# jason2714/de-i2i-gan

Hardware: AMD Instinct MI355X
Metric: paired 256x256 images/sec (G+D train step) (higher is better)
Workload: dtype bf16

## Files before the change

de-i2i-gan_amd/csrc/elementwise.hip:

```cpp
#include <hip/hip_runtime.h>
#include <algorithm>
#include <math.h>

#include "../../include/dei2i_hip.h"
#include "launch.h"

namespace dei2i {

template <typename T>
__global__ void nchw_to_nhwc_kernel(const float* __restrict__ src, T* __restrict__ dst, int N, int C, int hs, int ws, int H,
                                    int W, int Cs) {
  constexpr int VEC = Elem<T>::VEC;
  const int cv = Cs / VEC;
  const size_t total = (size_t)N * H * W * cv;
  for (size_t i = (size_t)blockIdx.x * blockDim.x + threadIdx.x; i < total; i += (size_t)gridDim.x * blockDim.x) {
    const size_t hw = (size_t)H * W;
    const size_t p = i % hw;
    size_t r = i / hw;
    const int v = (int)(r % cv);
    const int n = (int)(r / cv);
    const int h = (int)(p / W), w = (int)(p % W);
    const int sy = (int)(((long long)h * hs) / H), sx = (int)(((long long)w * ws) / W);
    float f[VEC];
#pragma unroll
// ... 54 lines not shown
    }
    const u32x4 pk = Elem<T>::pack(f);
    *reinterpret_cast<u32x4*>(out + i * VEC) = pk;
    if constexpr (sizeof(T) == 2) {
      if (out8 != nullptr) store_e4m3_of_bf16x8(out8 + i * 8, pk, scale8);
    }
  }
}

template <typename T>
__global__ void affine_act_img_kernel(const T* __restrict__ x, const float* __restrict__ A, const float* __restrict__ B,
                                      T* __restrict__ out, size_t nvec_img, int cv, float slope) {
  constexpr int VEC = Elem<T>::VEC;
  const int n = blockIdx.y;
  const size_t base = (size_t)n * nvec_img;
  float av[VEC], bv[VEC];
  size_t i = (size_t)blockIdx.x * blockDim.x + threadIdx.x;
  const int c = (int)(i % cv) * VEC;
  ldcoef<VEC>(A + (size_t)n * cv * VEC + c, av);
  ldcoef<VEC>(B + (size_t)n * cv * VEC + c, bv);
  for (; i < nvec_img; i += (size_t)gridDim.x * blockDim.x) {
    float f[VEC];
    Elem<T>::unpack(*reinterpret_cast<const u32x4*>(x + (base + i) * VEC), f);
#pragma unroll
    for (int e = 0; e < VEC; ++e) {
      const float v = fmaf(av[e], f[e], bv[e]);
      f[e] = fmaf(slope, fminf(v, 0.f), fmaxf(v, 0.f));
    }
    *reinterpret_cast<u32x4*>(out + (base + i) * VEC) = Elem<T>::pack(f);
  }
}


template <typename T>
__global__ void spade_act_kernel(const T* __restrict__ x, const float* __restrict__ mean, const float* __restrict__ rstd,
                                 const T* __restrict__ gb, T* __restrict__ out, int N, int H, int W, int C, int up,
                                 int gb_mode, unsigned char* __restrict__ out8, float scale8) {
  constexpr int VEC = Elem<T>::VEC;
  const int cv = C / VEC;
  const int Hs = H >> up, Ws = W >> up;
  const size_t total = (size_t)N * H * W * cv;
  for (size_t i = (size_t)blockIdx.x * blockDim.x + threadIdx.x; i < total; i += (size_t)gridDim.x * blockDim.x) {
    const int c = (int)(i % cv) * VEC;
    size_t r = i / cv;
    const int w = (int)(r % W); r /= W;
    const int h = (int)(r % H);
    const int n = (int)(r / H);
    float xv[VEC], gm[VEC], bt[VEC];
    Elem<T>::unpack(*reinterpret_cast<const u32x4*>(x + (((size_t)n * Hs + (h >> up)) * Ws + (w >> up)) * C + c), xv);
    size_t gpix;
    if (gb_mode == 0) gpix = ((size_t)n * H + h) * W + w;
    else gpix = ((size_t)n * 5 + border_class(h, H)) * 5 + border_class(w, W);
    Elem<T>::unpack(*reinterpret_cast<const u32x4*>(gb + gpix * 2 * C + c), gm);
    Elem<T>::unpack(*reinterpret_cast<const u32x4*>(gb + gpix * 2 * C + C + c), bt);
    float o[VEC], mv[VEC], rv[VEC];
    ldcoef<VEC>(mean + (size_t)n * C + c, mv);
    ldcoef<VEC>(rstd + (size_t)n * C + c, rv);
#pragma unroll
    for (int e = 0; e < VEC; ++e) {
      const float xh = (xv[e] - mv[e]) * rv[e];
      const float v = fmaf(xh, 1.f + gm[e], bt[e]);
      o[e] = v > 0.f ? v : 0.f;
    }
    const u32x4 pk = Elem<T>::pack(o);
    *reinterpret_cast<u32x4*>(out + i * VEC) = pk;
    if constexpr (sizeof(T) == 2) {
      if (out8 != nullptr) store_e4m3_of_bf16x8(out8 + i * 8, pk, scale8);
    }
  }
}

template <typename T>
__global__ void act_bwd_kernel(const T* __restrict__ dz, const T* __restrict__ z, T* __restrict__ g, size_t nvec, int act) {
  constexpr int VEC = Elem<T>::VEC;
  for (size_t i = (size_t)blockIdx.x * blockDim.x + threadIdx.x; i < nvec; i += (size_t)gridDim.x * blockDim.x) {
    float d[VEC], zz[VEC];
    Elem<T>::unpack(*reinterpret_cast<const u32x4*>(dz + i * VEC), d);
    Elem<T>::unpack(*reinterpret_cast<const u32x4*>(z + i * VEC), zz);
#pragma unroll
    for (int e = 0; e < VEC; ++e) d[e] *= act_grad_from_out(zz[e], act);
    *reinterpret_cast<u32x4*>(g + i * VEC) = Elem<T>::pack(d);
  }
}

template <typename T>
__global__ void compose_fwd_kernel(const T* __restrict__ raw, const float* __restrict__ x_in, float* __restrict__ out,
                                   float* __restrict__ prob, int N, int HW, int Cs) {
  const size_t total = (size_t)N * HW;
  for (size_t i = (size_t)blockIdx.x * blockDim.x + threadIdx.x; i < total; i += (size_t)gridDim.x * blockDim.x) {
    const size_t n = i / HW, p = i % HW;
    const T* rp = raw + i * Cs;
    const float pr = 1.f / (1.f + expf(-Elem<T>::load(rp + 3)));
    prob[i] = pr;
#pragma unroll
    for (int c = 0; c < 3; ++c) {
      const float fg = tanhf(Elem<T>::load(rp + c));
      const size_t o = (n * 3 + c) * HW + p;
      out[o] = x_in[o] * (1.f - pr) + fg * pr;
    }
  }
}

// ... 195 lines not shown
    else hipLaunchKernelGGL((affine_act_kernel<float, false>), dim3(grid, groups), dim3(256), 0, st, (const float*)x, a, b, (const float*)res, (float*)out, nvec, cv, act, o8, e4m3_scale);
  }
  return (int)hipGetLastError();
}

int dei2i_affine_act_img_fwd(int dtype, int N, int HW, int C, const void* x, const float* A, const float* B, float slope, void* out,
                             dei2i_stream s) {
  const int vec = vec_of(dtype);
  if (N <= 0 || HW <= 0 || C <= 0 || C % vec || !x || !A || !B || !out) return DEI2I_ERR_BAD_ARG;
  const int cv = C / vec;
  if (256 % cv != 0 && cv % 256 != 0) return DEI2I_ERR_BAD_ARG;
  const size_t nvec_img = (size_t)HW * cv;
  unsigned blocks = (unsigned)std::min<size_t>((nvec_img + 255) / 256, 512);
  if (cv > 256) blocks = (blocks / (cv / 256)) * (cv / 256);
  if (blocks < 1) blocks = cv > 256 ? cv / 256 : 1;
  if (dtype == DT_BF16)
    hipLaunchKernelGGL(affine_act_img_kernel<bf16_t>, dim3(blocks, N), dim3(256), 0, (hipStream_t)s, (const bf16_t*)x, A, B, (bf16_t*)out,
                       nvec_img, cv, slope);
  else
    hipLaunchKernelGGL(affine_act_img_kernel<float>, dim3(blocks, N), dim3(256), 0, (hipStream_t)s, (const float*)x, A, B, (float*)out,
                       nvec_img, cv, slope);
  return (int)hipGetLastError();
}

int dei2i_spade_act_fwd(int dtype, int N, int H, int W, int C, int up, const void* x, const float* mean, const float* rstd,
                        const void* gb, int gb_mode, void* out, void* out_e4m3, float e4m3_scale, dei2i_stream s) {
  const int vec = vec_of(dtype);
  if (N <= 0 || H <= 0 || W <= 0 || C <= 0 || C % vec || up < 0 || up > 1 || !x || !mean || !rstd || !gb || !out)
    return DEI2I_ERR_BAD_ARG;
  if (out_e4m3 != nullptr && (dtype != DT_BF16 || !(e4m3_scale > 0.f))) return DEI2I_ERR_BAD_ARG;
  unsigned char* o8 = (unsigned char*)out_e4m3;
  if (up && ((H | W) & 1)) return DEI2I_ERR_BAD_ARG;
  if (gb_mode == 1 && (H < 4 || W < 4)) return DEI2I_ERR_BAD_ARG;
  const size_t total = (size_t)N * H * W * (C / vec);
  if (dtype == DT_BF16)
    hipLaunchKernelGGL(spade_act_kernel<bf16_t>, dim3(grid_for(total, 256, EW_CAP)), dim3(256), 0, (hipStream_t)s,
                       (const bf16_t*)x, mean, rstd, (const bf16_t*)gb, (bf16_t*)out, N, H, W, C, up, gb_mode, o8, e4m3_scale);
  else
    hipLaunchKernelGGL(spade_act_kernel<float>, dim3(grid_for(total, 256, EW_CAP)), dim3(256), 0, (hipStream_t)s,
                       (const float*)x, mean, rstd, (const float*)gb, (float*)out, N, H, W, C, up, gb_mode, o8, e4m3_scale);
  return (int)hipGetLastError();
}

int dei2i_act_bwd(int dtype, size_t n, const void* dz, const void* z, int act, void* g, dei2i_stream s) {
  const int vec = vec_of(dtype);
  if (n == 0 || n % vec || !dz || !z || !g) return DEI2I_ERR_BAD_ARG;
  const size_t nvec = n / vec;
  if (dtype == DT_BF16)
    hipLaunchKernelGGL(act_bwd_kernel<bf16_t>, dim3(grid_for(nvec, 256, EW_CAP)), dim3(256), 0, (hipStream_t)s,
                       (const bf16_t*)dz, (const bf16_t*)z, (bf16_t*)g, nvec, act);
  else
    hipLaunchKernelGGL(act_bwd_kernel<float>, dim3(grid_for(nvec, 256, EW_CAP)), dim3(256), 0, (hipStream_t)s,
                       (const float*)dz, (const float*)z, (float*)g, nvec, act);
  return (int)hipGetLastError();
}

int dei2i_compose_fwd(int dtype, int N, int H, int W, int Cs, const void* raw, const float* x_in, float* out, float* prob,
                      dei2i_stream s) {
  if (N <= 0 || H <= 0 || W <= 0 || Cs < 4 || Cs % vec_of(dtype) || !raw || !x_in || !out || !prob) return DEI2I_ERR_BAD_ARG;
  const size_t total = (size_t)N * H * W;
  if (dtype == DT_BF16)
    hipLaunchKernelGGL(compose_fwd_kernel<bf16_t>, dim3(grid_for(total, 256, EW_CAP)), dim3(256), 0, (hipStream_t)s,
                       (const bf16_t*)raw, x_in, out, prob, N, H * W, Cs);
  else
    hipLaunchKernelGGL(compose_fwd_kernel<float>, dim3(grid_for(total, 256, EW_CAP)), dim3(256), 0, (hipStream_t)s,
                       (const float*)raw, x_in, out, prob, N, H * W, Cs);
  return (int)hipGetLastError();
}

int dei2i_compose_bwd(int dtype, int N, int H, int W, int Cs, const void* raw, const float* x_in, const float* d_out,
                      const float* d_prob, void* d_raw, float* d_x, dei2i_stream s) {
  if (N <= 0 || H <= 0 || W <= 0 || Cs < 4 || Cs % vec_of(dtype) || !raw || !x_in || !d_raw) return DEI2I_ERR_BAD_ARG;
  const size_t total = (size_t)N * H * W;
// ... 66 lines not shown
```

de-i2i-gan_amd/csrc/reduce.hip:

```cpp
#include <hip/hip_runtime.h>
#include <math.h>

#include "../../include/dei2i_hip.h"
#include "launch.h"

namespace dei2i {

static inline int vec_of(int dtype) { return dtype == DT_BF16 ? 8 : 4; }

template <int NV, int VEC, typename OT = float>
DEI2I_D void block_combine_store(const float (&vals)[NV][VEC], int cv, int rpp, float* smem, OT* __restrict__ dst, int C) {
  const int tid = threadIdx.x;
  const int vcol = tid % cv, prow = tid / cv;
  __syncthreads();
  if (prow < rpp) {
#pragma unroll
    for (int q = 0; q < NV; ++q)
#pragma unroll
      for (int e = 0; e < VEC; ++e) smem[((q * VEC + e) * rpp + prow) * cv + vcol] = vals[q][e];
  }
  __syncthreads();
#pragma unroll 1
  for (int o = tid; o < NV * VEC * cv; o += 256) {
    const int qe = o / cv, vc = o - qe * cv;
    const float* src = smem + (size_t)qe * rpp * cv + vc;
    float sum = 0.f;
    for (int r = 0; r < rpp; ++r) sum += src[r * cv];
    const int q = qe / VEC, e = qe - q * VEC;
    Elem<OT>::store(dst + (size_t)q * C + vc * VEC + e, sum);
  }
}

template <typename T>
// ... 374 lines not shown
        const float xh = (xv[e] - mv[e]) * rv[e];
        const float g = fmaf(xh, 1.f + gm[e], bt[e]) > 0.f ? d[e] : slope * d[e];
        v[0][e] = fmaf(g, xh, v[0][e]);
        v[1][e] += g;
      }
    }
  }
  block_combine_store<2, VEC, T>(v, cv, rpp, smem, dgb_cls + (((size_t)n * 5 + cy) * 5 + cx) * 2 * C, C);
}

__global__ __launch_bounds__(256) void spade_bwd_finalize_kernel(const float* __restrict__ partial, int N, int chunks, int C,
                                                                 double count, float* __restrict__ coef,
                                                                 void* __restrict__ dgb_cls, int dtype) {
  const int c = blockIdx.x, n = blockIdx.y;
  double sq[4];
  combine_records<4>(partial, (size_t)n * chunks, chunks, C, c, sq);
  if (threadIdx.x != 0) return;
  coef[((size_t)n * 2 + 0) * C + c] = (float)(sq[0] / count);
  coef[((size_t)n * 2 + 1) * C + c] = (float)(sq[1] / count);
  if (dgb_cls != nullptr) {
    const size_t gpix = ((size_t)n * 5 + 2) * 5 + 2;
    if (dtype == DT_BF16) {
      bf16_t* o = (bf16_t*)dgb_cls;
      o[gpix * 2 * C + c] = f32_to_bf16((float)sq[2]);
      o[gpix * 2 * C + C + c] = f32_to_bf16((float)sq[3]);
    } else {
      float* o = (float*)dgb_cls;
      o[gpix * 2 * C + c] = (float)sq[2];
      o[gpix * 2 * C + C + c] = (float)sq[3];
    }
  }
}

template <typename T>
__global__ void spade_bwd_apply_kernel(const T* __restrict__ dz, const T* __restrict__ x, const float* __restrict__ mean,
                                       const float* __restrict__ rstd, const T* __restrict__ gb, int gb_mode,
                                       const float* __restrict__ coef, const T* __restrict__ addend, T* __restrict__ dx, int N,
                                       int H, int W, int C, int up, float slope = 0.f) {
  constexpr int VEC = Elem<T>::VEC;
  const int cv = C / VEC;
  const int Hs = H >> up, Ws = W >> up;
  const size_t total = (size_t)N * Hs * Ws * cv;
  const float cnt = (float)(1 << (2 * up));
  for (size_t i = (size_t)blockIdx.x * blockDim.x + threadIdx.x; i < total; i += (size_t)gridDim.x * blockDim.x) {
    const int c = (int)(i % cv) * VEC;
    size_t r = i / cv;
    const int ws = (int)(r % Ws); r /= Ws;
    const int hs = (int)(r % Hs);
    const int n = (int)(r / Hs);
    float acc[VEC], xv[VEC], xh[VEC], mv[VEC], rv[VEC], k1[VEC], k2[VEC];
    ldcoef<VEC>(mean + (size_t)n * C + c, mv);
    ldcoef<VEC>(rstd + (size_t)n * C + c, rv);
    Elem<T>::unpack(*reinterpret_cast<const u32x4*>(x + i * VEC), xv);
#pragma unroll
    for (int e = 0; e < VEC; ++e) { acc[e] = 0.f; xh[e] = (xv[e] - mv[e]) * rv[e]; }
    for (int a = 0; a < (1 << up); ++a)
      for (int b = 0; b < (1 << up); ++b) {
        const int h = (hs << up) + a, w = (ws << up) + b;
        const size_t opix = ((size_t)n * H + h) * W + w;
        const size_t gpix = gb_mode == 0 ? opix : ((size_t)n * 5 + border_class(h, H)) * 5 + border_class(w, W);
        float d[VEC], gm[VEC], bt[VEC];
        Elem<T>::unpack(*reinterpret_cast<const u32x4*>(dz + opix * C + c), d);
        Elem<T>::unpack(*reinterpret_cast<const u32x4*>(gb + gpix * 2 * C + c), gm);
        Elem<T>::unpack(*reinterpret_cast<const u32x4*>(gb + gpix * 2 * C + C + c), bt);
#pragma unroll
        for (int e = 0; e < VEC; ++e) {
          const float g = fmaf(xh[e], 1.f + gm[e], bt[e]) > 0.f ? d[e] : slope * d[e];
          acc[e] = fmaf(g, 1.f + gm[e], acc[e]);
        }
      }
    float ad[VEC];
    if (addend != nullptr) Elem<T>::unpack(*reinterpret_cast<const u32x4*>(addend + i * VEC), ad);
    ldcoef<VEC>(coef + ((size_t)n * 2) * C + c, k1);
    ldcoef<VEC>(coef + ((size_t)n * 2 + 1) * C + c, k2);
#pragma unroll
    for (int e = 0; e < VEC; ++e) {
      float v = rv[e] * (acc[e] - cnt * k1[e] - cnt * xh[e] * k2[e]);
      if (addend != nullptr) v += ad[e];
      acc[e] = v;
    }
    *reinterpret_cast<u32x4*>(dx + i * VEC) = Elem<T>::pack(acc);
  }
}

template <typename T>
__global__ __launch_bounds__(256) void colsum_kernel(const T* __restrict__ g, float* __restrict__ partial, size_t rows, int C) {
  constexpr int VEC = Elem<T>::VEC;
  extern __shared__ float smem[];
  const int cv = C / VEC, rpp = 256 / cv;
  const int tid = threadIdx.x, vcol = tid % cv, prow = tid / cv;
  const size_t rows_per_block = (rows + gridDim.x - 1) / gridDim.x;
  const size_t rbeg = (size_t)blockIdx.x * rows_per_block;
  const size_t rend = rbeg + rows_per_block < rows ? rbeg + rows_per_block : rows;
  float v[1][VEC];
#pragma unroll
  for (int e = 0; e < VEC; ++e) v[0][e] = 0.f;
  if (prow < rpp) {
    const T* __restrict__ base = g + (size_t)vcol * VEC;
    auto acc = [&](const u32x4& q) {
      float f[VEC];
      Elem<T>::unpack(q, f);
#pragma unroll
      for (int e = 0; e < VEC; ++e) v[0][e] += f[e];
    };
    size_t r = rbeg + prow;
    for (; r + 3 * (size_t)rpp < rend; r += 4 * (size_t)rpp) {
      const u32x4 q0 = *reinterpret_cast<const u32x4*>(base + r * C);
      const u32x4 q1 = *reinterpret_cast<const u32x4*>(base + (r + rpp) * C);
      const u32x4 q2 = *reinterpret_cast<const u32x4*>(base + (r + 2 * (size_t)rpp) * C);
      const u32x4 q3 = *reinterpret_cast<const u32x4*>(base + (r + 3 * (size_t)rpp) * C);
      acc(q0); acc(q1); acc(q2); acc(q3);
    }
    for (; r < rend; r += rpp) acc(*reinterpret_cast<const u32x4*>(base + r * C));
  }
  block_combine_store<1, VEC>(v, cv, rpp, smem, partial + (size_t)blockIdx.x * C, C);
// ... 202 lines not shown
  if (ring == nullptr) return;
  const int H = Hs << up, W = Ws << up, cv = C / VEC;
  const int rp = ring_pixels(H, W);
  const int total = rp * cv;
  for (int i = blockIdx.x * 256 + tid; i < total; i += gridDim.x * 256) {
    const int r = i / cv, c = (i - r * cv) * VEC;
    int y, xx;
    ring_coord(r, H, W, y, xx);
    float xv[VEC], gm[VEC], bt[VEC], o[VEC];
    Elem<T>::unpack(*reinterpret_cast<const u32x4*>(x + (((size_t)n * Hs + (y >> up)) * Ws + (xx >> up)) * C + c), xv);
    const size_t gpix = ((size_t)n * 5 + prep_border_class(y, H)) * 5 + prep_border_class(xx, W);
    Elem<T>::unpack(*reinterpret_cast<const u32x4*>(gb + gpix * 2 * C + c), gm);
    Elem<T>::unpack(*reinterpret_cast<const u32x4*>(gb + gpix * 2 * C + C + c), bt);
#pragma unroll
    for (int e = 0; e < VEC; ++e) {
      const float xh = (xv[e] - smem[c + e]) * smem[C + c + e];
      const float v = fmaf(xh, 1.f + gm[e], bt[e]);
      o[e] = v > 0.f ? v : 0.f;
    }
    *reinterpret_cast<u32x4*>(ring + ((size_t)n * rp + r) * C + c) = Elem<T>::pack(o);
  }
}

}

using namespace dei2i;

static inline bool cv_ok(int dtype, int C) {
  const int vec = dtype == DT_BF16 ? 8 : 4;
  return C > 0 && C % vec == 0 && C / vec <= 256;
}
static inline size_t combine_lds(int dtype, int nv) { return (size_t)nv * (dtype == DT_BF16 ? 8 : 4) * 256 * sizeof(float); }

extern "C" {

int dei2i_moments_chunks(int HW) {
  int c = HW / 64;
  if (c < 1) c = 1;
  if (c > 64) c = 64;
  return c;
}

int dei2i_moments_partial(int dtype, int N, int HW, int C, const void* x, float* partial, dei2i_stream s) {
  if (N <= 0 || HW <= 0 || !cv_ok(dtype, C) || !x || !partial) return DEI2I_ERR_BAD_ARG;
  const int chunks = dei2i_moments_chunks(HW);
  if (dtype == DT_BF16)
    hipLaunchKernelGGL(moments_partial_kernel<bf16_t>, dim3(chunks, N), dim3(256), combine_lds(dtype, 2), (hipStream_t)s,
                       (const bf16_t*)x, partial, HW, C, chunks);
  else
    hipLaunchKernelGGL(moments_partial_kernel<float>, dim3(chunks, N), dim3(256), combine_lds(dtype, 2), (hipStream_t)s,
                       (const float*)x, partial, HW, C, chunks);
  return (int)hipGetLastError();
}

int dei2i_bn_finalize_train(int N, int HW, int C, const float* partial, const float* weight, const float* bias,
                            float* running_mean, float* running_var, float momentum, float eps, float* mean, float* rstd,
                            float* a, float* b, long long* num_batches_tracked, dei2i_stream s) {
  if (N <= 0 || HW <= 0 || C <= 0 || !partial || !weight || !bias || !mean || !rstd || !a || !b) return DEI2I_ERR_BAD_ARG;
  hipLaunchKernelGGL(bn_finalize_train_kernel, dim3(C), dim3(combine_threads(N * dei2i_moments_chunks(HW))), 0, (hipStream_t)s, partial, N,
                     dei2i_moments_chunks(HW), C, (double)N * (double)HW, weight, bias, running_mean, running_var, momentum,
                     eps, mean, rstd, a, b, num_batches_tracked, 0);
  return (int)hipGetLastError();
}

int dei2i_bn_finalize_train_chunks(int N, int HW, int C, int chunks, const float* partial, const float* weight, const float* bias,
                                   float* running_mean, float* running_var, float momentum, float eps, float* mean, float* rstd,
// ... 206 lines not shown
                       gb_mode == 0 ? (bf16_t*)dgb : (bf16_t*)nullptr, partial, H, W, C, up, chunks);
  else
    hipLaunchKernelGGL(spade_bwd_partial_kernel<float>, dim3(chunks, N), dim3(256), combine_lds(dtype, 4), st,
                       (const float*)dz, (const float*)x, mean, rstd, (const float*)gb, gb_mode,
                       gb_mode == 0 ? (float*)dgb : (float*)nullptr, partial, H, W, C, up, chunks);
  if (gb_mode == 1) {
    if (dtype == DT_BF16)
      hipLaunchKernelGGL(spade_bwd_border_kernel<bf16_t>, dim3(25, N), dim3(256), combine_lds(dtype, 2), st, (const bf16_t*)dz,
                         (const bf16_t*)x, mean, rstd, (const bf16_t*)gb, (bf16_t*)dgb, H, W, C, up);
    else
      hipLaunchKernelGGL(spade_bwd_border_kernel<float>, dim3(25, N), dim3(256), combine_lds(dtype, 2), st, (const float*)dz,
                         (const float*)x, mean, rstd, (const float*)gb, (float*)dgb, H, W, C, up);
  }
  return (int)hipGetLastError();
}

int dei2i_spade_bwd_border(int dtype, int N, int H, int W, int C, int up, const void* dz, const void* x, const float* mean,
                           const float* rstd, const void* gb, void* dgb_cls, dei2i_stream s) {
  if (N <= 0 || H < 4 || W < 4 || !cv_ok(dtype, C) || up < 0 || up > 1 || !dz || !x || !mean || !rstd || !gb || !dgb_cls)
    return DEI2I_ERR_BAD_ARG;
  hipStream_t st = (hipStream_t)s;
  if (dtype == DT_BF16)
    hipLaunchKernelGGL(spade_bwd_border_kernel<bf16_t>, dim3(25, N), dim3(256), combine_lds(dtype, 2), st, (const bf16_t*)dz,
                       (const bf16_t*)x, mean, rstd, (const bf16_t*)gb, (bf16_t*)dgb_cls, H, W, C, up);
  else
    hipLaunchKernelGGL(spade_bwd_border_kernel<float>, dim3(25, N), dim3(256), combine_lds(dtype, 2), st, (const float*)dz,
                       (const float*)x, mean, rstd, (const float*)gb, (float*)dgb_cls, H, W, C, up);
  return (int)hipGetLastError();
}

int dei2i_spade_bwd_apply(int dtype, int N, int H, int W, int C, int up, const void* dz, const void* x, const float* mean,
                          const float* rstd, const void* gb, int gb_mode, const float* partial, int chunks, void* dgb_cls,
                          float* coef, const void* addend, void* dx, dei2i_stream s) {
  const int vec = dtype == DT_BF16 ? 8 : 4;
  if (N <= 0 || H <= 0 || W <= 0 || !cv_ok(dtype, C) || up < 0 || up > 1 || !dz || !x || !mean || !rstd || !gb || !partial ||
      !coef || !dx)
    return DEI2I_ERR_BAD_ARG;
  hipStream_t st = (hipStream_t)s;
  hipLaunchKernelGGL(spade_bwd_finalize_kernel, dim3(C, N), dim3(combine_threads(chunks)), 0, st, partial, N, chunks, C,
                     (double)H * (double)W, coef, dgb_cls, dtype);
  const size_t total = (size_t)N * (H >> up) * (W >> up) * (C / vec);
  const unsigned grid = grid_for(total, 256, 256u * 16u);
  if (dtype == DT_BF16)
    hipLaunchKernelGGL(spade_bwd_apply_kernel<bf16_t>, dim3(grid), dim3(256), 0, st, (const bf16_t*)dz, (const bf16_t*)x, mean,
                       rstd, (const bf16_t*)gb, gb_mode, (const float*)coef, (const bf16_t*)addend, (bf16_t*)dx, N, H, W, C, up);
  else
    hipLaunchKernelGGL(spade_bwd_apply_kernel<float>, dim3(grid), dim3(256), 0, st, (const float*)dz, (const float*)x, mean,
                       rstd, (const float*)gb, gb_mode, (const float*)coef, (const float*)addend, (float*)dx, N, H, W, C, up);
  return (int)hipGetLastError();
}

int dei2i_in_act_bwd(int dtype, int N, int H, int W, int C, const void* dz, const void* x, const float* mean, const float* rstd,
                     float slope, const void* zero_table, float* partial, float* coef, const void* addend, void* dx, dei2i_stream s) {
  const int vec = dtype == DT_BF16 ? 8 : 4;
  if (N <= 0 || H < 4 || W < 4 || !cv_ok(dtype, C) || !dz || !x || !mean || !rstd || !zero_table || !partial || !coef || !dx)
    return DEI2I_ERR_BAD_ARG;
  hipStream_t st = (hipStream_t)s;
  const int chunks = dei2i_moments_chunks(H * W);
  if (dtype == DT_BF16)
    hipLaunchKernelGGL(spade_bwd_partial_kernel<bf16_t>, dim3(chunks, N), dim3(256), combine_lds(dtype, 4), st, (const bf16_t*)dz,
                       (const bf16_t*)x, mean, rstd, (const bf16_t*)zero_table, 1, (bf16_t*)nullptr, partial, H, W, C, 0, chunks, slope);
  else
    hipLaunchKernelGGL(spade_bwd_partial_kernel<float>, dim3(chunks, N), dim3(256), combine_lds(dtype, 4), st, (const float*)dz,
                       (const float*)x, mean, rstd, (const float*)zero_table, 1, (float*)nullptr, partial, H, W, C, 0, chunks, slope);
  hipLaunchKernelGGL(spade_bwd_finalize_kernel, dim3(C, N), dim3(combine_threads(chunks)), 0, st, (const float*)partial, N, chunks, C,
                     (double)H * (double)W, coef, (void*)nullptr, dtype);
  const size_t total = (size_t)N * H * W * (C / vec);
  const unsigned grid = grid_for(total, 256, 256u * 16u);
  if (dtype == DT_BF16)
    hipLaunchKernelGGL(spade_bwd_apply_kernel<bf16_t>, dim3(grid), dim3(256), 0, st, (const bf16_t*)dz, (const bf16_t*)x, mean, rstd,
                       (const bf16_t*)zero_table, 1, (const float*)coef, (const bf16_t*)addend, (bf16_t*)dx, N, H, W, C, 0, slope);
  else
    hipLaunchKernelGGL(spade_bwd_apply_kernel<float>, dim3(grid), dim3(256), 0, st, (const float*)dz, (const float*)x, mean, rstd,
                       (const float*)zero_table, 1, (const float*)coef, (const float*)addend, (float*)dx, N, H, W, C, 0, slope);
  return (int)hipGetLastError();
}

int dei2i_in_affine_act_bwd(int dtype, int N, int H, int W, int C, const void* dz, const void* x, const float* mean,
                            const float* rstd, float slope, const void* gb_table, void* dgb_table, float* partial, float* coef,
                            const void* addend, void* dx, dei2i_stream s) {
  const int vec = dtype == DT_BF16 ? 8 : 4;
  if (N <= 0 || H < 4 || W < 4 || !cv_ok(dtype, C) || !dz || !x || !mean || !rstd || !gb_table || !dgb_table || !partial || !coef || !dx)
    return DEI2I_ERR_BAD_ARG;
  hipStream_t st = (hipStream_t)s;
  const int chunks = dei2i_moments_chunks(H * W);
  const size_t total = (size_t)N * H * W * (C / vec);
  const unsigned grid = grid_for(total, 256, 256u * 16u);
  if (dtype == DT_BF16) {
    hipLaunchKernelGGL(spade_bwd_partial_kernel<bf16_t>, dim3(chunks, N), dim3(256), combine_lds(dtype, 4), st, (const bf16_t*)dz,
                       (const bf16_t*)x, mean, rstd, (const bf16_t*)gb_table, 1, (bf16_t*)nullptr, partial, H, W, C, 0, chunks, slope);
    hipLaunchKernelGGL(spade_bwd_border_kernel<bf16_t>, dim3(25, N), dim3(256), combine_lds(dtype, 2), st, (const bf16_t*)dz,
                       (const bf16_t*)x, mean, rstd, (const bf16_t*)gb_table, (bf16_t*)dgb_table, H, W, C, 0, slope);
  } else {
    hipLaunchKernelGGL(spade_bwd_partial_kernel<float>, dim3(chunks, N), dim3(256), combine_lds(dtype, 4), st, (const float*)dz,
                       (const float*)x, mean, rstd, (const float*)gb_table, 1, (float*)nullptr, partial, H, W, C, 0, chunks, slope);
    hipLaunchKernelGGL(spade_bwd_border_kernel<float>, dim3(25, N), dim3(256), combine_lds(dtype, 2), st, (const float*)dz,
                       (const float*)x, mean, rstd, (const float*)gb_table, (float*)dgb_table, H, W, C, 0, slope);
  }
  hipLaunchKernelGGL(spade_bwd_finalize_kernel, dim3(C, N), dim3(combine_threads(chunks)), 0, st, (const float*)partial, N, chunks, C,
                     (double)H * (double)W, coef, dgb_table, dtype);
  if (dtype == DT_BF16)
    hipLaunchKernelGGL(spade_bwd_apply_kernel<bf16_t>, dim3(grid), dim3(256), 0, st, (const bf16_t*)dz, (const bf16_t*)x, mean, rstd,
                       (const bf16_t*)gb_table, 1, (const float*)coef, (const bf16_t*)addend, (bf16_t*)dx, N, H, W, C, 0, slope);
  else
    hipLaunchKernelGGL(spade_bwd_apply_kernel<float>, dim3(grid), dim3(256), 0, st, (const float*)dz, (const float*)x, mean, rstd,
                       (const float*)gb_table, 1, (const float*)coef, (const float*)addend, (float*)dx, N, H, W, C, 0, slope);
  return (int)hipGetLastError();
}

__device__ float g_loss_partials[1024];

int dei2i_bce_logits_fwd(size_t n, const float* x, const float* target, float tconst, float* out, dei2i_stream s) {
  if (n == 0 || !x || !out) return DEI2I_ERR_BAD_ARG;
  hipStream_t st = (hipStream_t)s;
  float* part = nullptr;
  if (hipGetSymbolAddress((void**)&part, HIP_SYMBOL(g_loss_partials)) != hipSuccess) return DEI2I_ERR_BAD_ARG;
  const unsigned nb = grid_for(n, 256, 1024);
  hipLaunchKernelGGL(bce_fwd_kernel, dim3(nb), dim3(256), 0, st, x, target, tconst, n, 1.f / (float)n, part);
  hipLaunchKernelGGL(loss_finalize_kernel, dim3(1), dim3(256), 0, st, (const float*)part, (int)nb, 1.f / (float)n, out, 0);
  return (int)hipGetLastError();
}

int dei2i_bce_logits_bwd(size_t n, const float* x, const float* target, float tconst, const float* gout, float* dx,
                         dei2i_stream s) {
  if (n == 0 || !x || !gout || !dx) return DEI2I_ERR_BAD_ARG;
  hipLaunchKernelGGL(bce_bwd_kernel, dim3(grid_for(n, 256, 1024)), dim3(256), 0, (hipStream_t)s, x, target, tconst, n,
                     1.f / (float)n, gout, dx);
  return (int)hipGetLastError();
}

int dei2i_l1_fwd(size_t n, const float* a, const float* b, float* out, dei2i_stream s) {
  if (n == 0 || !a || !out) return DEI2I_ERR_BAD_ARG;
  hipStream_t st = (hipStream_t)s;
  float* part = nullptr;
  if (hipGetSymbolAddress((void**)&part, HIP_SYMBOL(g_loss_partials)) != hipSuccess) return DEI2I_ERR_BAD_ARG;
  const unsigned nb = grid_for(n, 256, 1024);
  hipLaunchKernelGGL(l1_fwd_kernel, dim3(nb), dim3(256), 0, st, a, b, n, 1.f / (float)n, part);
  hipLaunchKernelGGL(loss_finalize_kernel, dim3(1), dim3(256), 0, st, (const float*)part, (int)nb, 1.f / (float)n, out, 0);
  return (int)hipGetLastError();
}
// ... 39 lines not shown
```

Measured before the change: 474.5.

## Restructure SPADE act forward and backward-apply kernels into per-image channel-tiled runs

```diff
diff --git a/de-i2i-gan_amd/csrc/elementwise.hip b/de-i2i-gan_amd/csrc/elementwise.hip
--- a/de-i2i-gan_amd/csrc/elementwise.hip
+++ b/de-i2i-gan_amd/csrc/elementwise.hip
@@ -110,30 +110,50 @@
 }
 
 
-template <typename T>
-__global__ void spade_act_kernel(const T* __restrict__ x, const float* __restrict__ mean, const float* __restrict__ rstd,
-                                 const T* __restrict__ gb, T* __restrict__ out, int N, int H, int W, int C, int up,
-                                 int gb_mode, unsigned char* __restrict__ out8, float scale8) {
-  constexpr int VEC = Elem<T>::VEC;
-  const int cv = C / VEC;
-  const int Hs = H >> up, Ws = W >> up;
-  const size_t total = (size_t)N * H * W * cv;
-  for (size_t i = (size_t)blockIdx.x * blockDim.x + threadIdx.x; i < total; i += (size_t)gridDim.x * blockDim.x) {
-    const int c = (int)(i % cv) * VEC;
-    size_t r = i / cv;
-    const int w = (int)(r % W); r /= W;
-    const int h = (int)(r % H);
-    const int n = (int)(r / H);
-    float xv[VEC], gm[VEC], bt[VEC];
-    Elem<T>::unpack(*reinterpret_cast<const u32x4*>(x + (((size_t)n * Hs + (h >> up)) * Ws + (w >> up)) * C + c), xv);
-    size_t gpix;
-    if (gb_mode == 0) gpix = ((size_t)n * H + h) * W + w;
-    else gpix = ((size_t)n * 5 + border_class(h, H)) * 5 + border_class(w, W);
-    Elem<T>::unpack(*reinterpret_cast<const u32x4*>(gb + gpix * 2 * C + c), gm);
-    Elem<T>::unpack(*reinterpret_cast<const u32x4*>(gb + gpix * 2 * C + C + c), bt);
-    float o[VEC], mv[VEC], rv[VEC];
-    ldcoef<VEC>(mean + (size_t)n * C + c, mv);
-    ldcoef<VEC>(rstd + (size_t)n * C + c, rv);
+template <typename T, int UP>
+__global__ __launch_bounds__(256) void spade_act_kernel(const T* __restrict__ x, const float* __restrict__ mean,
+                                                        const float* __restrict__ rstd, const T* __restrict__ gb, T* __restrict__ out,
+                                                        int H, int W, int C, FastDiv w_div, int run, int gb_mode,
+                                                        unsigned char* __restrict__ out8, float scale8) {
+  constexpr int VEC = Elem<T>::VEC, U = 4;
+  const int cv = C / VEC, rpp = 256 / cv;
+  const int tid = threadIdx.x, vcol = tid % cv, prow = tid / cv;
+  if (prow >= rpp) return;
+  const int n = blockIdx.y, c = vcol * VEC;
+  const int HW = H * W, Ws = W >> UP;
+  const int pbeg = blockIdx.x * run, pend = min(HW, pbeg + run);
+  const size_t out_img = (size_t)n * HW * C;
+  const T* __restrict__ xb = x + (size_t)n * (H >> UP) * Ws * C + c;
+  T* __restrict__ ob = out + out_img + c;
+  const T* __restrict__ gbb = gb + (gb_mode == 0 ? out_img * 2 : (size_t)n * 25 * 2 * C) + c;
+  float mv[VEC], rv[VEC];
+  ldcoef<VEC>(mean + (size_t)n * C + c, mv);
+  ldcoef<VEC>(rstd + (size_t)n * C + c, rv);
+  u32x4 gmi = {0u, 0u, 0u, 0u}, bti = {0u, 0u, 0u, 0u};
+  if (gb_mode != 0) {
+    gmi = *reinterpret_cast<const u32x4*>(gbb + 12 * 2 * C);
+    bti = *reinterpret_cast<const u32x4*>(gbb + 12 * 2 * C + C);
+  }
+  struct Pix { u32x4 x, gm, bt; int p; };
+  auto load = [&](int p) {
+    Pix q;
+    q.p = p;
+    const int h = (int)fd_div((uint32_t)p, w_div), w = p - h * W;
+    q.x = *reinterpret_cast<const u32x4*>(xb + ((h >> UP) * Ws + (w >> UP)) * C);
+    q.gm = gmi; q.bt = bti;
+    if (gb_mode == 0) {
+      q.gm = *reinterpret_cast<const u32x4*>(gbb + p * 2 * C);
+      q.bt = *reinterpret_cast<const u32x4*>(gbb + p * 2 * C + C);
+    } else if (h < 2 || h >= H - 2 || w < 2 || w >= W - 2) {
+      const int o = (border_class(h, H) * 5 + border_class(w, W)) * 2 * C;
+      q.gm = *reinterpret_cast<const u32x4*>(gbb + o);
+      q.bt = *reinterpret_cast<const u32x4*>(gbb + o + C);
+    }
+    return q;
+  };
+  auto use = [&](const Pix& q) {
+    float xv[VEC], gm[VEC], bt[VEC], o[VEC];
+    Elem<T>::unpack(q.x, xv); Elem<T>::unpack(q.gm, gm); Elem<T>::unpack(q.bt, bt);
 #pragma unroll
     for (int e = 0; e < VEC; ++e) {
       const float xh = (xv[e] - mv[e]) * rv[e];
@@ -141,11 +161,20 @@
       o[e] = v > 0.f ? v : 0.f;
     }
     const u32x4 pk = Elem<T>::pack(o);
-    *reinterpret_cast<u32x4*>(out + i * VEC) = pk;
+    *reinterpret_cast<u32x4*>(ob + q.p * C) = pk;
     if constexpr (sizeof(T) == 2) {
-      if (out8 != nullptr) store_e4m3_of_bf16x8(out8 + i * 8, pk, scale8);
-    }
-  }
+      if (out8 != nullptr) store_e4m3_of_bf16x8(out8 + out_img + c + (size_t)q.p * C, pk, scale8);
+    }
+  };
+  int p = pbeg + prow;
+  for (; p + (U - 1) * rpp < pend; p += U * rpp) {
+    Pix q[U];
+#pragma unroll
+    for (int k = 0; k < U; ++k) q[k] = load(p + k * rpp);
+#pragma unroll
+    for (int k = 0; k < U; ++k) use(q[k]);
+  }
+  for (; p < pend; p += rpp) use(load(p));
 }
 
 template <typename T>
@@ -407,13 +436,24 @@
   unsigned char* o8 = (unsigned char*)out_e4m3;
   if (up && ((H | W) & 1)) return DEI2I_ERR_BAD_ARG;
   if (gb_mode == 1 && (H < 4 || W < 4)) return DEI2I_ERR_BAD_ARG;
-  const size_t total = (size_t)N * H * W * (C / vec);
-  if (dtype == DT_BF16)
-    hipLaunchKernelGGL(spade_act_kernel<bf16_t>, dim3(grid_for(total, 256, EW_CAP)), dim3(256), 0, (hipStream_t)s,
-                       (const bf16_t*)x, mean, rstd, (const bf16_t*)gb, (bf16_t*)out, N, H, W, C, up, gb_mode, o8, e4m3_scale);
-  else
-    hipLaunchKernelGGL(spade_act_kernel<float>, dim3(grid_for(total, 256, EW_CAP)), dim3(256), 0, (hipStream_t)s,
-                       (const float*)x, mean, rstd, (const float*)gb, (float*)out, N, H, W, C, up, gb_mode, o8, e4m3_scale);
+  if ((size_t)H * W * 2 * C >= (1ull << 31) || C / vec > 256) return DEI2I_ERR_BAD_ARG;
+  const int cv = C / vec, rpp = 256 / cv, HW = H * W, unit = rpp * 4;
+  int blocks = (HW + unit - 1) / unit, run = unit;
+  const int cap = std::max(1, 4096 / N);
+  if (blocks > cap) {
+    run = (HW + cap - 1) / cap;
+    run = (run + unit - 1) / unit * unit;
+    blocks = (HW + run - 1) / run;
+  }
+  const FastDiv wd = make_fastdiv((uint32_t)W);
+  const dim3 grid(blocks, N);
+  hipStream_t st = (hipStream_t)s;
+#define DEI2I_SA(TY, UPV)                                                                                                    \
+  hipLaunchKernelGGL((spade_act_kernel<TY, UPV>), grid, dim3(256), 0, st, (const TY*)x, mean, rstd, (const TY*)gb, (TY*)out, H, W, C, \
+                     wd, run, gb_mode, o8, e4m3_scale)
+  if (dtype == DT_BF16) { if (up) DEI2I_SA(bf16_t, 1); else DEI2I_SA(bf16_t, 0); }
+  else { if (up) DEI2I_SA(float, 1); else DEI2I_SA(float, 0); }
+#undef DEI2I_SA
   return (int)hipGetLastError();
 }
 
diff --git a/de-i2i-gan_amd/csrc/reduce.hip b/de-i2i-gan_amd/csrc/reduce.hip
--- a/de-i2i-gan_amd/csrc/reduce.hip
+++ b/de-i2i-gan_amd/csrc/reduce.hip
@@ -1,4 +1,5 @@
 #include <hip/hip_runtime.h>
+#include <algorithm>
 #include <math.h>
 
 #include "../../include/dei2i_hip.h"
@@ -439,37 +440,78 @@
   }
 }
 
-template <typename T>
-__global__ void spade_bwd_apply_kernel(const T* __restrict__ dz, const T* __restrict__ x, const float* __restrict__ mean,
-                                       const float* __restrict__ rstd, const T* __restrict__ gb, int gb_mode,
-                                       const float* __restrict__ coef, const T* __restrict__ addend, T* __restrict__ dx, int N,
-                                       int H, int W, int C, int up, float slope = 0.f) {
-  constexpr int VEC = Elem<T>::VEC;
-  const int cv = C / VEC;
-  const int Hs = H >> up, Ws = W >> up;
-  const size_t total = (size_t)N * Hs * Ws * cv;
-  const float cnt = (float)(1 << (2 * up));
-  for (size_t i = (size_t)blockIdx.x * blockDim.x + threadIdx.x; i < total; i += (size_t)gridDim.x * blockDim.x) {
-    const int c = (int)(i % cv) * VEC;
-    size_t r = i / cv;
-    const int ws = (int)(r % Ws); r /= Ws;
-    const int hs = (int)(r % Hs);
-    const int n = (int)(r / Hs);
-    float acc[VEC], xv[VEC], xh[VEC], mv[VEC], rv[VEC], k1[VEC], k2[VEC];
-    ldcoef<VEC>(mean + (size_t)n * C + c, mv);
-    ldcoef<VEC>(rstd + (size_t)n * C + c, rv);
-    Elem<T>::unpack(*reinterpret_cast<const u32x4*>(x + i * VEC), xv);
+template <typename T, int UP>
+__global__ __launch_bounds__(256) void spade_bwd_apply_kernel(const T* __restrict__ dz, const T* __restrict__ x,
+                                                              const float* __restrict__ mean, const float* __restrict__ rstd,
+                                                              const T* __restrict__ gb, int gb_mode, const float* __restrict__ coef,
+                                                              const T* __restrict__ addend, T* __restrict__ dx, int H, int W, int C,
+                                                              FastDiv ws_div, int run, float slope) {
+  constexpr int VEC = Elem<T>::VEC, U = 2;
+  constexpr int CELL = 1 << UP;
+  const int cv = C / VEC, rpp = 256 / cv;
+  const int tid = threadIdx.x, vcol = tid % cv, prow = tid / cv;
+  if (prow >= rpp) return;
+  const int n = blockIdx.y, c = vcol * VEC;
+  const int Hs = H >> UP, Ws = W >> UP, P = Hs * Ws;
+  const int pbeg = blockIdx.x * run, pend = min(P, pbeg + run);
+  const float cnt = (float)(1 << (2 * UP));
+  const size_t src_img = (size_t)n * P * C, out_img = (size_t)n * H * W * C;
+  const T* __restrict__ xb = x + src_img + c;
+  const T* __restrict__ ab = addend != nullptr ? addend + src_img + c : nullptr;
+  T* __restrict__ db = dx + src_img + c;
+  const T* __restrict__ dzb = dz + out_img + c;
+  const T* __restrict__ gbb = gb + (gb_mode == 0 ? out_img * 2 : (size_t)n * 25 * 2 * C) + c;
+  float mv[VEC], rv[VEC], k1[VEC], k2[VEC];
+  ldcoef<VEC>(mean + (size_t)n * C + c, mv);
+  ldcoef<VEC>(rstd + (size_t)n * C + c, rv);
+  ldcoef<VEC>(coef + ((size_t)n * 2) * C + c, k1);
+  ldcoef<VEC>(coef + ((size_t)n * 2 + 1) * C + c, k2);
+  u32x4 gmi = {0u, 0u, 0u, 0u}, bti = {0u, 0u, 0u, 0u};
+  if (gb_mode != 0) {
+    gmi = *reinterpret_cast<const u32x4*>(gbb + 12 * 2 * C);
+    bti = *reinterpret_cast<const u32x4*>(gbb + 12 * 2 * C + C);
+  }
+
+  struct Pix { u32x4 x, ad, d[CELL][CELL]; int p, h0, w0; };
+  auto load = [&](int p) {
+    Pix q;
+    q.p = p;
+    const int hs = (int)fd_div((uint32_t)p, ws_div), wsrc = p - hs * Ws;
+    q.h0 = hs << UP; q.w0 = wsrc << UP;
+    q.x = *reinterpret_cast<const u32x4*>(xb + p * C);
+    if (ab != nullptr) q.ad = *reinterpret_cast<const u32x4*>(ab + p * C);
+#pragma unroll
+    for (int a = 0; a < CELL; ++a) {
+      const T* row = dzb + ((q.h0 + a) * W + q.w0) * C;
+#pragma unroll
+      for (int b = 0; b < CELL; ++b) q.d[a][b] = *reinterpret_cast<const u32x4*>(row + b * C);
+    }
+    return q;
+  };
+  auto use = [&](const Pix& q) {
+    float acc[VEC], xv[VEC], xh[VEC];
+    Elem<T>::unpack(q.x, xv);
 #pragma unroll
     for (int e = 0; e < VEC; ++e) { acc[e] = 0.f; xh[e] = (xv[e] - mv[e]) * rv[e]; }
-    for (int a = 0; a < (1 << up); ++a)
-      for (int b = 0; b < (1 << up); ++b) {
-        const int h = (hs << up) + a, w = (ws << up) + b;
-        const size_t opix = ((size_t)n * H + h) * W + w;
-        const size_t gpix = gb_mode == 0 ? opix : ((size_t)n * 5 + border_class(h, H)) * 5 + border_class(w, W);
+#pragma unroll
+    for (int a = 0; a < CELL; ++a)
+#pragma unroll
+      for (int b = 0; b < CELL; ++b) {
+        const int h = q.h0 + a, w = q.w0 + b;
+        u32x4 gq = gmi, bq = bti;
+        if (gb_mode == 0) {
+          const int o = (h * W + w) * 2 * C;
+          gq = *reinterpret_cast<const u32x4*>(gbb + o);
+          bq = *reinterpret_cast<const u32x4*>(gbb + o + C);
+        } else if (h < 2 || h >= H - 2 || w < 2 || w >= W - 2) {
+          const int o = (border_class(h, H) * 5 + border_class(w, W)) * 2 * C;
+          gq = *reinterpret_cast<const u32x4*>(gbb + o);
+          bq = *reinterpret_cast<const u32x4*>(gbb + o + C);
+        }
         float d[VEC], gm[VEC], bt[VEC];
-        Elem<T>::unpack(*reinterpret_cast<const u32x4*>(dz + opix * C + c), d);
-        Elem<T>::unpack(*reinterpret_cast<const u32x4*>(gb + gpix * 2 * C + c), gm);
-        Elem<T>::unpack(*reinterpret_cast<const u32x4*>(gb + gpix * 2 * C + C + c), bt);
+        Elem<T>::unpack(q.d[a][b], d);
+        Elem<T>::unpack(gq, gm);
+        Elem<T>::unpack(bq, bt);
 #pragma unroll
         for (int e = 0; e < VEC; ++e) {
           const float g = fmaf(xh[e], 1.f + gm[e], bt[e]) > 0.f ? d[e] : slope * d[e];
@@ -477,17 +519,24 @@
         }
       }
     float ad[VEC];
-    if (addend != nullptr) Elem<T>::unpack(*reinterpret_cast<const u32x4*>(addend + i * VEC), ad);
-    ldcoef<VEC>(coef + ((size_t)n * 2) * C + c, k1);
-    ldcoef<VEC>(coef + ((size_t)n * 2 + 1) * C + c, k2);
+    if (ab != nullptr) Elem<T>::unpack(q.ad, ad);
 #pragma unroll
     for (int e = 0; e < VEC; ++e) {
       float v = rv[e] * (acc[e] - cnt * k1[e] - cnt * xh[e] * k2[e]);
-      if (addend != nullptr) v += ad[e];
+      if (ab != nullptr) v += ad[e];
       acc[e] = v;
     }
-    *reinterpret_cast<u32x4*>(dx + i * VEC) = Elem<T>::pack(acc);
-  }
+    *reinterpret_cast<u32x4*>(db + q.p * C) = Elem<T>::pack(acc);
+  };
+  int p = pbeg + prow;
+  for (; p + (U - 1) * rpp < pend; p += U * rpp) {
+    Pix q[U];
+#pragma unroll
+    for (int k = 0; k < U; ++k) q[k] = load(p + k * rpp);
+#pragma unroll
+    for (int k = 0; k < U; ++k) use(q[k]);
+  }
+  for (; p < pend; p += rpp) use(load(p));
 }
 
 template <typename T>
@@ -756,6 +805,32 @@
 }
 static inline size_t combine_lds(int dtype, int nv) { return (size_t)nv * (dtype == DT_BF16 ? 8 : 4) * 256 * sizeof(float); }
 
+static int launch_spade_bwd_apply(int dtype, int N, int H, int W, int C, int up, const void* dz, const void* x, const float* mean,
+                                  const float* rstd, const void* gb, int gb_mode, const float* coef, const void* addend, void* dx,
+                                  float slope, hipStream_t st) {
+  if ((size_t)H * W * 2 * C >= (1ull << 31)) return DEI2I_ERR_BAD_ARG;
+  const int cv = C / (dtype == DT_BF16 ? 8 : 4), rpp = 256 / cv;
+  const int Hs = H >> up, Ws = W >> up, P = Hs * Ws;
+  if (P == 0) return DEI2I_ERR_BAD_ARG;
+  const int unit = rpp * 4;
+  int blocks = (P + unit - 1) / unit, run = unit;
+  const int cap = std::max(1, 4096 / N);
+  if (blocks > cap) {
+    run = (P + cap - 1) / cap;
+    run = (run + unit - 1) / unit * unit;
+    blocks = (P + run - 1) / run;
+  }
+  const FastDiv wd = make_fastdiv((uint32_t)Ws);
+  const dim3 grid(blocks, N);
+#define DEI2I_SBA(TY, UPV)                                                                                                  \
+  hipLaunchKernelGGL((spade_bwd_apply_kernel<TY, UPV>), grid, dim3(256), 0, st, (const TY*)dz, (const TY*)x, mean, rstd,    \
+                     (const TY*)gb, gb_mode, coef, (const TY*)addend, (TY*)dx, H, W, C, wd, run, slope)
+  if (dtype == DT_BF16) { if (up) DEI2I_SBA(bf16_t, 1); else DEI2I_SBA(bf16_t, 0); }
+  else { if (up) DEI2I_SBA(float, 1); else DEI2I_SBA(float, 0); }
+#undef DEI2I_SBA
+  return (int)hipGetLastError();
+}
+
 extern "C" {
 
 int dei2i_moments_chunks(int HW) {
@@ -1028,27 +1103,17 @@
 int dei2i_spade_bwd_apply(int dtype, int N, int H, int W, int C, int up, const void* dz, const void* x, const float* mean,
                           const float* rstd, const void* gb, int gb_mode, const float* partial, int chunks, void* dgb_cls,
                           float* coef, const void* addend, void* dx, dei2i_stream s) {
-  const int vec = dtype == DT_BF16 ? 8 : 4;
   if (N <= 0 || H <= 0 || W <= 0 || !cv_ok(dtype, C) || up < 0 || up > 1 || !dz || !x || !mean || !rstd || !gb || !partial ||
       !coef || !dx)
     return DEI2I_ERR_BAD_ARG;
   hipStream_t st = (hipStream_t)s;
   hipLaunchKernelGGL(spade_bwd_finalize_kernel, dim3(C, N), dim3(combine_threads(chunks)), 0, st, partial, N, chunks, C,
                      (double)H * (double)W, coef, dgb_cls, dtype);
-  const size_t total = (size_t)N * (H >> up) * (W >> up) * (C / vec);
-  const unsigned grid = grid_for(total, 256, 256u * 16u);
-  if (dtype == DT_BF16)
-    hipLaunchKernelGGL(spade_bwd_apply_kernel<bf16_t>, dim3(grid), dim3(256), 0, st, (const bf16_t*)dz, (const bf16_t*)x, mean,
-                       rstd, (const bf16_t*)gb, gb_mode, (const float*)coef, (const bf16_t*)addend, (bf16_t*)dx, N, H, W, C, up);
-  else
-    hipLaunchKernelGGL(spade_bwd_apply_kernel<float>, dim3(grid), dim3(256), 0, st, (const float*)dz, (const float*)x, mean,
-                       rstd, (const float*)gb, gb_mode, (const float*)coef, (const float*)addend, (float*)dx, N, H, W, C, up);
-  return (int)hipGetLastError();
+  return launch_spade_bwd_apply(dtype, N, H, W, C, up, dz, x, mean, rstd, gb, gb_mode, coef, addend, dx, 0.f, st);
 }
 
 int dei2i_in_act_bwd(int dtype, int N, int H, int W, int C, const void* dz, const void* x, const float* mean, const float* rstd,
                      float slope, const void* zero_table, float* partial, float* coef, const void* addend, void* dx, dei2i_stream s) {
-  const int vec = dtype == DT_BF16 ? 8 : 4;
   if (N <= 0 || H < 4 || W < 4 || !cv_ok(dtype, C) || !dz || !x || !mean || !rstd || !zero_table || !partial || !coef || !dx)
     return DEI2I_ERR_BAD_ARG;
   hipStream_t st = (hipStream_t)s;
@@ -1061,27 +1126,16 @@
                        (const float*)x, mean, rstd, (const float*)zero_table, 1, (float*)nullptr, partial, H, W, C, 0, chunks, slope);
   hipLaunchKernelGGL(spade_bwd_finalize_kernel, dim3(C, N), dim3(combine_threads(chunks)), 0, st, (const float*)partial, N, chunks, C,
                      (double)H * (double)W, coef, (void*)nullptr, dtype);
-  const size_t total = (size_t)N * H * W * (C / vec);
-  const unsigned grid = grid_for(total, 256, 256u * 16u);
-  if (dtype == DT_BF16)
-    hipLaunchKernelGGL(spade_bwd_apply_kernel<bf16_t>, dim3(grid), dim3(256), 0, st, (const bf16_t*)dz, (const bf16_t*)x, mean, rstd,
-                       (const bf16_t*)zero_table, 1, (const float*)coef, (const bf16_t*)addend, (bf16_t*)dx, N, H, W, C, 0, slope);
-  else
-    hipLaunchKernelGGL(spade_bwd_apply_kernel<float>, dim3(grid), dim3(256), 0, st, (const float*)dz, (const float*)x, mean, rstd,
-                       (const float*)zero_table, 1, (const float*)coef, (const float*)addend, (float*)dx, N, H, W, C, 0, slope);
-  return (int)hipGetLastError();
+  return launch_spade_bwd_apply(dtype, N, H, W, C, 0, dz, x, mean, rstd, zero_table, 1, coef, addend, dx, slope, st);
 }
 
 int dei2i_in_affine_act_bwd(int dtype, int N, int H, int W, int C, const void* dz, const void* x, const float* mean,
                             const float* rstd, float slope, const void* gb_table, void* dgb_table, float* partial, float* coef,
                             const void* addend, void* dx, dei2i_stream s) {
-  const int vec = dtype == DT_BF16 ? 8 : 4;
   if (N <= 0 || H < 4 || W < 4 || !cv_ok(dtype, C) || !dz || !x || !mean || !rstd || !gb_table || !dgb_table || !partial || !coef || !dx)
     return DEI2I_ERR_BAD_ARG;
   hipStream_t st = (hipStream_t)s;
   const int chunks = dei2i_moments_chunks(H * W);
-  const size_t total = (size_t)N * H * W * (C / vec);
-  const unsigned grid = grid_for(total, 256, 256u * 16u);
   if (dtype == DT_BF16) {
     hipLaunchKernelGGL(spade_bwd_partial_kernel<bf16_t>, dim3(chunks, N), dim3(256), combine_lds(dtype, 4), st, (const bf16_t*)dz,
                        (const bf16_t*)x, mean, rstd, (const bf16_t*)gb_table, 1, (bf16_t*)nullptr, partial, H, W, C, 0, chunks, slope);
@@ -1095,13 +1149,7 @@
   }
   hipLaunchKernelGGL(spade_bwd_finalize_kernel, dim3(C, N), dim3(combine_threads(chunks)), 0, st, (const float*)partial, N, chunks, C,
                      (double)H * (double)W, coef, dgb_table, dtype);
-  if (dtype == DT_BF16)
-    hipLaunchKernelGGL(spade_bwd_apply_kernel<bf16_t>, dim3(grid), dim3(256), 0, st, (const bf16_t*)dz, (const bf16_t*)x, mean, rstd,
-                       (const bf16_t*)gb_table, 1, (const float*)coef, (const bf16_t*)addend, (bf16_t*)dx, N, H, W, C, 0, slope);
-  else
-    hipLaunchKernelGGL(spade_bwd_apply_kernel<float>, dim3(grid), dim3(256), 0, st, (const float*)dz, (const float*)x, mean, rstd,
-                       (const float*)gb_table, 1, (const float*)coef, (const float*)addend, (float*)dx, N, H, W, C, 0, slope);
-  return (int)hipGetLastError();
+  return launch_spade_bwd_apply(dtype, N, H, W, C, 0, dz, x, mean, rstd, gb_table, 1, coef, addend, dx, slope, st);
 }
 
 __device__ float g_loss_partials[1024];
```

Result: no change. 479.2 (median of 6 runs) (+1.0%).
